# clawrim/gcn10

Hardware: AMD Instinct MI355X
Metric: CN Gpixels/sec (higher is better)
Workload: dtype u8

## Files before the change

### gcn10_amd/csrc/gcn10_gpu.hip

```cpp

#include <hip/hip_runtime.h>
#include <unistd.h>
#include <hip/hip_ext.h>

#include <cstdarg>
#include <cstdint>
#include <cstdio>
#include <cstdlib>
#include <cstring>
#include <new>

#include "gcn10_gpu.h"
#include "gcn10_gpu_internal.hpp"
#include "gcn10_soil_readers.hpp"

using gcn10::as_stream;
using gcn10::fail;
using gcn10::kLut16Bytes;
using gcn10::kLut16Plane;
using gcn10::kPlanes;
using gcn10::SoilView;
using gcn10::u32x4;
using gcn10::use_device;

namespace {

constexpr int kThreads = 256;
constexpr int kPxPerLane = 16;
constexpr int kChunk = kThreads * kPxPerLane;
constexpr int kInvalidPlane = kPlanes - 1;
constexpr int kPlane1 = 256 + 4;
constexpr int kLut1Bytes = kPlanes * kPlane1;


struct StripParams {
    const uint8_t *esa;
    SoilView soil;
    const uint8_t *lut;
    uint8_t *out[GCN10_N_RASTERS];
    uint32_t W;
    uint32_t rows;
    uint32_t npix;
    uint32_t nvec16;
    uint32_t nchunks;
    uint32_t table_mask;
    uint32_t single_k;
    uint32_t xcd_slabs;
    const uint32_t *cx;
    const uint8_t *codes;
    uint32_t codes_stride;
    const uint32_t *soil_complex;
    uint32_t soil_gen;
};

__host__ __device__ inline uint8_t soil_code(uint8_t h)
{
    uint8_t d, u;
    if (h >= 11 && h <= 14) {
        d = 4;
        u = (uint8_t)(h - 10);
    }
    else {
        d = u = (h < 5) ? h : (uint8_t)kInvalidPlane;
    }
    return (uint8_t)(d | (u << 4));
}


__device__ __forceinline__ u32x4 load16_aligned_nt(const uint8_t *p)
{
    return __builtin_nontemporal_load(reinterpret_cast<const u32x4 *>(p));
}

__device__ __forceinline__ u32x4 load16_aligned(const uint8_t *p)
{
    return *reinterpret_cast<const u32x4 *>(p);
}

__device__ __forceinline__ u32x4 load16_any(const uint8_t *p)
{
    typedef u32x4 u32x4_u __attribute__((aligned(1)));
    return *reinterpret_cast<const u32x4_u *>(p);
}

template <bool NT = true>
__device__ __forceinline__ void store16(uint8_t *p, u32x4 v)
{
    if (NT)
        __builtin_nontemporal_store(v, reinterpret_cast<u32x4 *>(p));
    else
        *reinterpret_cast<u32x4 *>(p) = v;
}

__device__ __forceinline__ int32_t scalar_load_i32(const int32_t *base, uint32_t i)
{
    typedef const int32_t __attribute__((address_space(4))) *const_ptr_t;
    const_ptr_t cp = (const_ptr_t)(uintptr_t)base;
    return cp[__builtin_amdgcn_readfirstlane(i)];
}

__device__ __forceinline__ uint32_t first_chunk(uint32_t nchunks, uint32_t &step,
                                                uint32_t &end, bool xcd_slabs)
{
    uint32_t nb = gridDim.x;
    uint32_t b = blockIdx.x;
    if (xcd_slabs && nb % 8u == 0u && nchunks >= nb) {
        uint32_t xcd = b & 7u;
        uint32_t per = (nchunks + 7u) / 8u;
        uint32_t lo = xcd * per;
        uint32_t hi = lo + per < nchunks ? lo + per : nchunks;
        step = nb / 8u;
        end = hi;
        return lo + (b >> 3);
    }
    step = nb;
    end = nchunks;
    return b;
}

enum { kLut16 = 0, kLut1 = 1 };
constexpr uint32_t kWavePx = 64u * kPxPerLane;
constexpr uint32_t kMinVectorW = kWavePx + 16u;

enum { kSoilBytes = 0, kSoilLanes = 1, kSoilPixels = 2 };

template <int ILP>
struct Trip {
    u32x4 e16[ILP], c16[ILP];
    uint32_t i0[ILP];
};

template <int ILP, bool NT>
__device__ __forceinline__ void issue_trip(const StripParams &p, uint32_t trip, uint32_t lane_off,
                                           uint32_t wave_off, Trip<ILP> &tr)
{
    uint32_t xb[ILP], r0[ILP], r1[ILP], wb[ILP];
#pragma unroll
    for (int u = 0; u < ILP; u++) {
        wb[u] = __builtin_amdgcn_readfirstlane((trip * ILP + u) * (uint32_t)kChunk + wave_off);
        const uint32_t wbc = wb[u] < p.npix ? wb[u] : 0u;
        const uint32_t y = wbc / p.W;
        xb[u] = wbc - y * p.W;
        r0[u] = (uint32_t)scalar_load_i32(p.soil.cj, y);
        r1[u] = (uint32_t)scalar_load_i32(p.soil.cj, y + 1u < p.rows ? y + 1u : y);
    }
#pragma unroll
    for (int u = 0; u < ILP; u++) {
        tr.i0[u] = wb[u] + lane_off;
        const uint8_t *pe = p.esa + (tr.i0[u] < p.nvec16 ? tr.i0[u] : 0u);
        tr.e16[u] = NT ? load16_aligned_nt(pe) : load16_aligned(pe);
    }
#pragma unroll
    for (int u = 0; u < ILP; u++) {
        uint32_t xl = xb[u] + lane_off;
        const bool wrap = xl >= p.W;
        xl = wrap ? xl - p.W : xl;
        const uint32_t row = p.soil.clamp(wrap ? r1[u] : r0[u]);
        const uint8_t *pa = p.soil.at(row, xl);
        u32x4 a = load16_any(pa);
        if (p.W & 15u) {
            const uint32_t n = p.W - xl;
            const bool strad = !wrap && n < (uint32_t)kPxPerLane;
            if (__builtin_amdgcn_ballot_w64(strad) != 0ull) {
                const uint8_t *pb = strad ? p.soil.at(p.soil.clamp(r1[u]), 0u) - n : pa;
                const u32x4 b = load16_any(pb);
                const uint32_t nn = strad ? n : (uint32_t)kPxPerLane;
#pragma unroll
                for (int j = 0; j < 4; j++) {
                    const int32_t m = (int32_t)nn - 4 * j;
                    const uint32_t mask = m >= 4 ? 0xffffffffu : (m <= 0 ? 0u : (1u << (8 * m)) - 1u);
                    a[j] = (a[j] & mask) | (b[j] & ~mask);
                }
            }
        }
        tr.c16[u] = a;
    }
}

struct LaneSoil {
    uint32_t base;
    uint32_t lim;
    uint32_t sub_px;
    uint32_t y_first;
    uint32_t B;
    bool wrap;
    uint32_t x;
    uint32_t c_lo, c_hi;
    int32_t split;
    uint32_t mask[4];
    bool pair;
};

__device__ __forceinline__ uint32_t split_mask(int32_t split, int j)
{
    const int32_t m = split - 4 * j;
    return m >= 4 ? 0xffffffffu : (m <= 0 ? 0u : (1u << (8 * m)) - 1u);
}

template <int SOIL>
__device__ __forceinline__ void lane_prologue(const StripParams &p, const gcn10::StripLanePlan &pl, LaneSoil &ls)
{
    const uint32_t g_first = __builtin_amdgcn_readfirstlane(pl.g);
    ls.base = (pl.row_lo * pl.G + pl.t) * (uint32_t)kPxPerLane;
    ls.lim = pl.active ? pl.row_hi * p.W : 0u;
    ls.sub_px = pl.B * p.W;
    ls.y_first = pl.row_lo + __builtin_amdgcn_readfirstlane(pl.rho);
    ls.B = pl.B;
    ls.wrap = pl.g < g_first;
    ls.x = pl.g * (uint32_t)kPxPerLane;
    ls.c_lo = ls.c_hi = 0u;
    ls.split = 16;
    ls.pair = true;
    if (SOIL == kSoilLanes) {
        uint32_t cx[16];
#pragma unroll
        for (int j = 0; j < 4; j++) {
            const u32x4 c4 = *reinterpret_cast<const u32x4 *>(p.cx + ls.x + 4 * j);
#pragma unroll
            for (int q = 0; q < 4; q++)
                cx[4 * j + q] = c4[q];
        }
        ls.c_lo = cx[0];
        ls.c_hi = cx[15];
        uint32_t split = 0;
#pragma unroll
        for (int q = 0; q < 16; q++)
            split += cx[q] == ls.c_lo && split == (uint32_t)q ? 1u : 0u;
        ls.split = (int32_t)split;
#pragma unroll
        for (int j = 0; j < 4; j++)
            ls.mask[j] = split_mask(ls.split, j);
        ls.pair = __builtin_amdgcn_ballot_w64(ls.c_hi - ls.c_lo > 1u) == 0ull;
    }
}

template <int ILP, bool NT, int SOIL>
__device__ __forceinline__ void issue_lane_trip(const StripParams &p, const LaneSoil &ls, uint32_t trip,
                                                Trip<ILP> &tr)
{
    uint32_t o0[ILP], o1[ILP];
#pragma unroll
    for (int u = 0; u < ILP; u++) {
        const uint32_t y = ls.y_first + (trip * ILP + u) * ls.B;
        const uint32_t ya = y < p.rows ? y : p.rows - 1u;
        const uint32_t yb = y + 1u < p.rows ? y + 1u : p.rows - 1u;
        o0[u] = p.soil.clamp((uint32_t)scalar_load_i32(p.soil.cj, ya)) * p.codes_stride;
        o1[u] = p.soil.clamp((uint32_t)scalar_load_i32(p.soil.cj, yb)) * p.codes_stride;
    }
#pragma unroll
    for (int u = 0; u < ILP; u++) {
        const uint32_t i0 = ls.base + (trip * ILP + u) * ls.sub_px;
        const bool live = i0 < ls.lim;
        tr.i0[u] = live ? i0 : 0xffffffffu;
        const uint8_t *pe = p.esa + (live ? i0 : 0u);
        tr.e16[u] = NT ? load16_aligned_nt(pe) : load16_aligned(pe);
    }
#pragma unroll
    for (int u = 0; u < ILP; u++) {
        const uint32_t off = ls.wrap ? o1[u] : o0[u];
        if (SOIL == kSoilLanes) {
            typedef uint16_t u16_u __attribute__((aligned(1)));
            tr.c16[u][0] = *reinterpret_cast<const u16_u *>(p.codes + (off + ls.c_lo));
            if (!ls.pair)
                tr.c16[u][1] = p.codes[off + ls.c_hi];
        }
        else {
            const uint8_t *cr = p.codes + off;
            const u32x4 *pc = reinterpret_cast<const u32x4 *>(p.cx + ls.x);
            u32x4 a = { 0u, 0u, 0u, 0u };
#pragma unroll 1
            for (int j = 0; j < 4; j++) {
                const u32x4 c4 = pc[j];
                const uint32_t w = (uint32_t)cr[c4[0]] | (uint32_t)cr[c4[1]] << 8 | (uint32_t)cr[c4[2]] << 16 |
                                   (uint32_t)cr[c4[3]] << 24;
                a[0] = j == 0 ? w : a[0];
                a[1] = j == 1 ? w : a[1];
                a[2] = j == 2 ? w : a[2];
                a[3] = j == 3 ? w : a[3];
            }
            tr.c16[u] = a;
        }
    }
}

template <bool KEEP_MASKS>
__device__ __forceinline__ u32x4 mix_lane_codes(const LaneSoil &ls, const u32x4 &c)
{
    const uint32_t a = (c[0] & 0xffu) * 0x01010101u;
    const uint32_t b = (ls.pair ? (c[0] >> 8) & 0xffu : c[1] & 0xffu) * 0x01010101u;
    u32x4 cd;
    int32_t split = ls.split;
    if (!KEEP_MASKS)
        asm volatile("" : "+v"(split));
#pragma unroll
    for (int j = 0; j < 4; j++) {
        const uint32_t mask = KEEP_MASKS ? ls.mask[j] : split_mask(split, j);
        cd[j] = (a & mask) | (b & ~mask);
    }
    return cd;
}

template <int KIND, int COND_MASK, int ILP, bool NT, int SOIL>
__device__ __forceinline__ void finish_trip(const StripParams &p, const uint8_t *lut, uint32_t tmask,
                                            const Trip<ILP> &tr, const LaneSoil &ls)
{
#pragma unroll
    for (int u = 0; u < ILP; u++) {
        const bool live = tr.i0[u] < p.nvec16;
        const u32x4 c16 = SOIL == kSoilLanes ? mix_lane_codes<KIND == kLut1>(ls, tr.c16[u]) : tr.c16[u];
#pragma unroll
        for (int c = 0; c < 2; c++) {
            if (!(COND_MASK & (1 << c)))
                continue;
            if (KIND == kLut16) {
                uint32_t acc[9][4];
                gcn10::gather16(lut, tr.e16[u], c16, c, acc);
                if (live) {
#pragma unroll
                    for (int k = 0; k < 9; k++) {
                        if (tmask & (1u << k)) {
                            u32x4 v = {acc[k][0], acc[k][1], acc[k][2], acc[k][3]};
                            store16<NT>(p.out[c * 9 + k] + tr.i0[u], v);
                        }
                    }
                }
            }
            else {
                u32x4 v;
#pragma unroll
                for (int j = 0; j < 4; j++) {
                    const uint32_t e = tr.e16[u][j];
                    const uint32_t cd = c16[j];
                    uint32_t w = 0;
#pragma unroll
                    for (int q = 0; q < 4; q++) {
                        const uint32_t lc = (e >> (8 * q)) & 0xffu;
                        const uint32_t s = (cd >> (8 * q + 4 * c)) & 0xfu;
                        const uint32_t b = lut[s * (uint32_t)kPlane1 + lc];
                        w |= b << (8 * q);
                    }
                    v[j] = w;
                }
                if (live)
                    store16<NT>(p.out[c * 9 + p.single_k] + tr.i0[u], v);
            }
        }
    }
}

template <int KIND, int COND_MASK, int ILP, bool NT, bool PF, int SOIL>
__device__ __forceinline__ void strip_loop(const StripParams &p, const uint8_t *lut, uint32_t tmask)
{
    uint32_t step = 1u, end, trip = 0u, lane_off = 0u, wave_off = 0u;
    LaneSoil ls = {};
    if (SOIL == kSoilBytes) {
        lane_off = (threadIdx.x & 63u) * kPxPerLane;
        wave_off = __builtin_amdgcn_readfirstlane(threadIdx.x >> 6) * kWavePx;
        trip = first_chunk(p.nchunks, step, end, p.xcd_slabs != 0);
    }
    else {
        const gcn10::StripLanePlan pl = gcn10::strip_lane_plan(p.W, p.rows, gridDim.x, blockIdx.x, threadIdx.x,
                                                               p.xcd_slabs != 0, (uint32_t)ILP);
        end = __builtin_amdgcn_readfirstlane(pl.trips);
        if (!__builtin_amdgcn_readfirstlane((uint32_t)pl.active))
            return;
        lane_prologue<SOIL>(p, pl, ls);
    }
    if (trip >= end)
        return;
    auto issue = [&](uint32_t t, Trip<ILP> &tr) {
        if (SOIL == kSoilBytes)
            issue_trip<ILP, NT>(p, t, lane_off, wave_off, tr);
        else
            issue_lane_trip<ILP, NT, SOIL>(p, ls, t, tr);
    };
    if (!PF) {
        for (; trip < end; trip += step) {
            Trip<ILP> tr;
            issue(trip, tr);
            finish_trip<KIND, COND_MASK, ILP, NT, SOIL>(p, lut, tmask, tr, ls);
        }
    }
    else {
        Trip<ILP> ta, tb;
        issue(trip, ta);
        for (;;) {
            trip += step;
            if (trip >= end) {
                finish_trip<KIND, COND_MASK, ILP, NT, SOIL>(p, lut, tmask, ta, ls);
                break;
            }
            issue(trip, tb);
            finish_trip<KIND, COND_MASK, ILP, NT, SOIL>(p, lut, tmask, ta, ls);
            trip += step;
            if (trip >= end) {
                finish_trip<KIND, COND_MASK, ILP, NT, SOIL>(p, lut, tmask, tb, ls);
                break;
            }
            issue(trip, ta);
            finish_trip<KIND, COND_MASK, ILP, NT, SOIL>(p, lut, tmask, tb, ls);
        }
    }
}

template <int KIND, int COND_MASK, bool ALL_TABLES, int ILP, bool NT, bool PF>
__global__ __launch_bounds__(kThreads) void cn_strip_kernel(const StripParams p)
{
    constexpr int kLutBytes = KIND == kLut16 ? kLut16Bytes : kLut1Bytes;
    __shared__ __attribute__((aligned(16))) uint8_t lut[kLutBytes];

    if (KIND == kLut16) {
        gcn10::stage_lut16<kThreads>(lut, p.lut);
    }
    else {
        const uint32_t *src = reinterpret_cast<const uint32_t *>(p.lut);
        uint32_t *dst = reinterpret_cast<uint32_t *>(lut);
        for (int i = threadIdx.x; i < kLutBytes / 4; i += kThreads)
            dst[i] = src[i];
    }
    __syncthreads();

    const uint32_t tmask = ALL_TABLES ? 0x1ffu : p.table_mask;

    if (!p.codes)
        strip_loop<KIND, COND_MASK, ILP, NT, PF, kSoilBytes>(p, lut, tmask);
    else if ((uint32_t)scalar_load_i32(reinterpret_cast<const int32_t *>(p.soil_complex), 0u) != p.soil_gen)
        strip_loop<KIND, COND_MASK, ILP, NT, PF, kSoilLanes>(p, lut, tmask);
    else
        strip_loop<KIND, COND_MASK, ILP, NT, PF, kSoilPixels>(p, lut, tmask);

    if (blockIdx.x == 0 && threadIdx.x < p.npix - p.nvec16) {
        const uint32_t i = p.nvec16 + threadIdx.x;
        const uint32_t y = i / p.W;
        const uint32_t x = i - y * p.W;
        const uint32_t lc = p.esa[i];
        const uint32_t cd = *p.soil.ptr(y, x);
#pragma unroll
        for (int c = 0; c < 2; c++) {
            if (!(COND_MASK & (1 << c)))
                continue;
            const uint32_t s = (cd >> (4 * c)) & 0xfu;
            if (KIND == kLut16) {
                const uint8_t *row = gcn10::lut16_row(lut, s, lc);
                for (int k = 0; k < 9; k++)
                    if (tmask & (1u << k))
                        p.out[c * 9 + k][i] = row[k];
            }
            else {
                p.out[c * 9 + p.single_k][i] = lut[s * (uint32_t)kPlane1 + lc];
            }
        }
    }
}

__global__ __launch_bounds__(kThreads) void stream_copy_kernel(const u32x4 *in, u32x4 *out, uint32_t nvec,
                                                               uint32_t ntrips)
{
    uint32_t step, end;
    for (uint32_t trip = first_chunk(ntrips, step, end, true); trip < end; trip += step) {
        u32x4 v[2];
        uint32_t idx[2];
#pragma unroll
        for (int u = 0; u < 2; u++) {
            idx[u] = (trip * 2u + u) * (uint32_t)kThreads + threadIdx.x;
            v[u] = __builtin_nontemporal_load(in + (idx[u] < nvec ? idx[u] : 0u));
        }
#pragma unroll
        for (int u = 0; u < 2; u++)
            if (idx[u] < nvec)
                __builtin_nontemporal_store(v[u], out + idx[u]);
    }
}

__global__ __launch_bounds__(kThreads) void cn_strip_bytes(const StripParams p,
                                                           uint32_t cond_mask)
{
    __shared__ __attribute__((aligned(16))) uint8_t lut[kLut16Bytes];
    gcn10::stage_lut16<kThreads>(lut, p.lut);
    __syncthreads();

    const uint32_t stride = gridDim.x * blockDim.x;
    for (uint32_t i = blockIdx.x * blockDim.x + threadIdx.x; i < p.npix; i += stride) {
        const uint32_t y = i / p.W;
        const uint32_t x = i - y * p.W;
        const uint32_t lc = p.esa[i];
        const uint32_t cd = *p.soil.ptr(y, x);
        for (int c = 0; c < 2; c++) {
            if (!(cond_mask & (1u << c)))
                continue;
            const uint32_t s = (cd >> (4 * c)) & 0xfu;
            const uint8_t *row = gcn10::lut16_row(lut, s, lc);
            for (int k = 0; k < 9; k++)
                if (p.table_mask & (1u << k))
                    p.out[c * 9 + k][i] = row[k];
        }
    }
}

template <bool VEC>
__global__ __launch_bounds__(kThreads) void soil_tables_kernel(const uint8_t *coarse, uint32_t hsx, uint32_t hsy,
                                                               const int32_t *ci, uint32_t W, uint32_t hx_stride,
                                                               uint8_t *codes, uint32_t codes_stride,
                                                               uint32_t *cx_out, uint32_t *complex, uint32_t gen)
{
    const uint32_t pad = (uint32_t)(kInvalidPlane | (kInvalidPlane << 4));
    if (blockIdx.y >= 1u) {
        const uint32_t per_row = codes_stride / 16u;
        const uint32_t t = ((blockIdx.y - 1u) * gridDim.x + blockIdx.x) * blockDim.x + threadIdx.x;
        const uint32_t r = t / per_row;
        if (r >= hsy)
            return;
        const uint32_t c0 = (t - r * per_row) * 16u;
        const uint8_t *row = coarse + (size_t)r * hsx;
        u32x4 in = { 0u, 0u, 0u, 0u };
        if (c0 + 16u <= hsx) {
            in = load16_any(row + c0);
        }
        else {
#pragma unroll
            for (int q = 0; q < 16; q++)
                if (c0 + q < hsx)
                    in[q >> 2] |= (uint32_t)row[c0 + q] << (8 * (q & 3));
        }
        u32x4 o;
#pragma unroll
        for (int j = 0; j < 4; j++) {
            uint32_t w = 0;
#pragma unroll
            for (int q = 0; q < 4; q++) {
                const uint32_t code = c0 + 4 * j + q < hsx ? soil_code((uint8_t)(in[j] >> (8 * q))) : pad;
                w |= code << (8 * q);
            }
            o[j] = w;
        }
        *reinterpret_cast<u32x4 *>(codes + (size_t)r * codes_stride + c0) = o;
        return;
    }
    const uint32_t x = (blockIdx.x * blockDim.x + threadIdx.x) * 16u;
    if (x >= hx_stride)
        return;
    uint32_t cx[16];
    if (VEC && x + 16u <= W) {
        const u32x4 *civ = reinterpret_cast<const u32x4 *>(ci + x);
#pragma unroll
        for (int j = 0; j < 4; j++) {
            const u32x4 c4 = civ[j];
#pragma unroll
            for (int q = 0; q < 4; q++)
                cx[4 * j + q] = c4[q] < hsx ? c4[q] : hsx - 1u;
        }
    }
    else {
#pragma unroll
        for (int q = 0; q < 16; q++) {
            const uint32_t xx = x + q;
            const uint32_t c = xx < W ? (uint32_t)ci[xx] : 0u;
            cx[q] = xx < W ? (c < hsx ? c : hsx - 1u) : hsx;
        }
    }
    const uint32_t c_lo = cx[0], c_hi = cx[15];
    uint32_t split = 0;
    bool compact = true;
#pragma unroll
    for (int q = 0; q < 16; q++) {
        const bool lo = cx[q] == c_lo;
        compact = compact && (lo ? split == (uint32_t)q : cx[q] == c_hi);
        split += lo && split == (uint32_t)q ? 1u : 0u;
    }
#pragma unroll
    for (int j = 0; j < 4; j++)
        *reinterpret_cast<u32x4 *>(cx_out + x + 4 * j) =
            u32x4{ cx[4 * j], cx[4 * j + 1], cx[4 * j + 2], cx[4 * j + 3] };
    if (x < W && !compact && *reinterpret_cast<volatile uint32_t *>(complex) != gen)
        *reinterpret_cast<volatile uint32_t *>(complex) = gen;
}

constexpr uint32_t kExpandRows = 4;

__global__ __launch_bounds__(kThreads) void expand_code_bytes(const uint8_t *codes, uint32_t codes_stride,
                                                              uint32_t hsy, const uint32_t *cx_in, uint8_t *hx,
                                                              uint32_t hx_stride)
{
// ... 799 lines not shown
    if (npix == 0)
        return GCN10_OK;
    if (!esa || !hsg || !out)
        return fail(GCN10_E_INVAL, "gcn10_gpu_calculate_cn: null pointer");
    const uint8_t *img = ctx->d_lut1 + (size_t)table_index * kLut1Bytes;
    const bool vec = aligned16(esa) && aligned16(hsg) && aligned16(out);
    const uint64_t work = vec ? (npix / 16 + 2 * kThreads - 1) / (2 * kThreads) + 1
                              : (npix + kThreads - 1) / kThreads;
    const uint32_t grid = stream_grid(ctx, work);
    if (vec)
        hipLaunchKernelGGL(calculate_cn_kernel<true>, dim3(grid), dim3(kThreads), 0,
                           as_stream(ctx, stream), esa, hsg, npix, img, out);
    else
        hipLaunchKernelGGL(calculate_cn_kernel<false>, dim3(grid), dim3(kThreads), 0,
                           as_stream(ctx, stream), esa, hsg, npix, img, out);
    HIP_TRY(hipGetLastError());
    return GCN10_OK;
}


int gcn10_gpu_prepare_tile(gcn10_gpu_ctx *ctx, const uint8_t *coarse, int hsx, int hsy,
                           const int32_t *ci, int W, gcn10_stream_t stream)
{
    int rc = use_device(ctx);
    if (rc)
        return rc;
    if (hsx <= 0 || hsy <= 0 || W <= 0)
        return fail(GCN10_E_INVAL, "gcn10_gpu_prepare_tile: bad shape W=%d soil=%dx%d", W, hsx, hsy);
    if (!coarse || !ci)
        return fail(GCN10_E_INVAL, "gcn10_gpu_prepare_tile: null pointer");
    const uint32_t stride = (((uint32_t)W + 15u) & ~15u) + 16u;
    const size_t need_hx = ((size_t)stride * (size_t)hsy + 63) & ~(size_t)63;
    const uint32_t codes_stride = (((uint32_t)hsx + 1u) + 15u) & ~15u;
    const size_t off_cx = (need_hx + 15) & ~(size_t)15;
    const size_t off_codes = (off_cx + (size_t)stride * 4u + 15) & ~(size_t)15;
    const size_t need = off_codes + (size_t)codes_stride * (size_t)hsy;
    if (need > ctx->hx_capacity) {
        HIP_TRY(hipDeviceSynchronize());
        if (ctx->d_hx_alloc)
            HIP_TRY(hipFree(ctx->d_hx_alloc));
        ctx->d_hx_alloc = ctx->d_hx = nullptr;
        ctx->hx_capacity = 0;
        ctx->hx_W = 0;
        HIP_TRY(hipMalloc(reinterpret_cast<void **>(&ctx->d_hx_alloc), 16 + need));
        ctx->d_hx = ctx->d_hx_alloc + 16;
        ctx->hx_capacity = need;
    }
    ctx->d_cx = reinterpret_cast<uint32_t *>(ctx->d_hx + off_cx);
    ctx->d_codes = ctx->d_hx + off_codes;
    ctx->codes_stride = codes_stride;
    if (++ctx->soil_gen == 0u)
        ctx->soil_gen = 1u;
    ctx->hx_made = false;
    ctx->hx_stride = stride;
    ctx->hx_W = (uint32_t)W;
    ctx->hx_rows = (uint32_t)hsy;
    hipStream_t s = as_stream(ctx, stream);
    const uint32_t group_blocks = (stride / 16u + kThreads - 1) / kThreads;
    const size_t code_threads = (size_t)(codes_stride / 16u) * (size_t)hsy;
    const uint32_t code_chunks = (uint32_t)((code_threads + (size_t)group_blocks * kThreads - 1) / ((size_t)group_blocks * kThreads));
    auto fn = aligned16(ci) ? soil_tables_kernel<true> : soil_tables_kernel<false>;
    hipLaunchKernelGGL(fn, dim3(group_blocks, 1u + code_chunks), dim3(kThreads), 0, s, coarse, (uint32_t)hsx,
                       (uint32_t)hsy, ci, (uint32_t)W, stride, ctx->d_codes, codes_stride, ctx->d_cx,
                       ctx->d_soil_complex, ctx->soil_gen);
    HIP_TRY(hipGetLastError());
    if (!ctx->compact_soil || (W & 15)) {
        const uint8_t *hx;
        return gcn10::soil_bytes(ctx, s, &hx);
    }
    return GCN10_OK;
}

int gcn10_gpu_cn_strip(gcn10_gpu_ctx *ctx, const uint8_t *esa, int W, int rows,
                       const int32_t *cj, unsigned cond_mask, unsigned table_mask,
                       uint8_t *const out[GCN10_N_RASTERS], gcn10_stream_t stream)
{
    int rc = use_device(ctx);
    if (rc)
        return rc;
    const char *const who = "gcn10_gpu_cn_strip";
    if ((rc = gcn10::check_tables(ctx, who)) != GCN10_OK || (rc = gcn10::check_tile(ctx, who)) != GCN10_OK)
        return rc;
    if (W <= 0 || rows < 0 || (uint32_t)W != ctx->hx_W)
        return fail(GCN10_E_INVAL, "gcn10_gpu_cn_strip: W=%d rows=%d does not match prepared tile W=%u",
                    W, rows, ctx->hx_W);
    if ((uint64_t)W * (uint64_t)rows > 0x7fffffffull)
        return fail(GCN10_E_INVAL, "gcn10_gpu_cn_strip: strip of %d x %d exceeds 2^31-1 pixels", W, rows);
    if ((rc = gcn10::check_masks(ctx, who, cond_mask, table_mask)) != GCN10_OK)
        return rc;
    if (rows == 0)
        return GCN10_OK;
    if (!esa || !cj || !out)
        return fail(GCN10_E_INVAL, "gcn10_gpu_cn_strip: null pointer");

    StripParams p;
    memset(&p, 0, sizeof p);
    bool all_aligned = aligned16(esa);
    for (int r = 0; r < GCN10_N_RASTERS; r++) {
        if (!gcn10::selected(r, cond_mask, table_mask))
            continue;
        if (!out[r])
            return fail(GCN10_E_INVAL, "gcn10_gpu_cn_strip: out[%d] is null but selected", r);
        p.out[r] = out[r];
        all_aligned = all_aligned && aligned16(out[r]);
    }
    p.esa = esa;
    p.W = (uint32_t)W;
    p.rows = (uint32_t)rows;
    p.npix = (uint32_t)((uint64_t)W * (uint64_t)rows);
    p.nchunks = (p.npix + kChunk - 1) / kChunk;
    p.table_mask = table_mask;
    hipStream_t s = as_stream(ctx, stream);

    p.xcd_slabs = (uint32_t)ctx->xcd_slabs;
    p.nvec16 = p.npix & ~15u;
    if (p.npix < 16u || p.W < kMinVectorW)
        all_aligned = false;
    const bool single = popcount(table_mask) == 1;
    const bool tuned = single && ctx->single.set;
    const int n_streams = popcount(cond_mask) * popcount(table_mask);
    const int ilp = tuned ? ctx->single.ilp
                          : single ? ctx->ilp1 : (ctx->ilp16 > 0 ? ctx->ilp16 : (n_streams > 9 ? 1 : 2));
    p.nchunks = (p.nchunks + (uint32_t)ilp - 1) / (uint32_t)ilp;
    const uint32_t grid = stream_grid(ctx, p.nchunks, tuned ? ctx->single.grid_blocks_per_cu : 0);
    if (tuned)
        p.xcd_slabs = (uint32_t)ctx->single.xcd_slabs;
    if (all_aligned && ctx->compact_soil && (p.W & 15u) == 0u &&
        gcn10::strip_lane_plan(p.W, p.rows, grid, 0u, 0u, p.xcd_slabs != 0, (uint32_t)ilp).B > 0u) {
        p.soil = SoilView{ nullptr, cj, ctx->hx_stride, ctx->hx_rows };
        p.cx = ctx->d_cx;
        p.codes = ctx->d_codes;
        p.codes_stride = ctx->codes_stride;
        p.soil_complex = ctx->d_soil_complex;
        p.soil_gen = ctx->soil_gen;
    }
    else {
        rc = gcn10::bind_soil(ctx, who, W, s, cj, &p.soil);
        if (rc)
            return rc;
    }
    if (!all_aligned) {
        p.lut = ctx->d_lut16;
        const uint32_t g = stream_grid(ctx, ((uint64_t)p.npix + kThreads - 1) / kThreads);
        void *args[] = { &p, &cond_mask };
        HIP_TRY(launch_timed(ctx, reinterpret_cast<const void *>(cn_strip_bytes), g, args, s));
        ctx->last_kernel = "cn_strip_bytes";
    }
    else {
        const bool all = table_mask == 0x1ffu;
        const bool nt = ctx->nontemporal != 0;
        if (single) {
            p.single_k = (uint32_t)__builtin_ctz(table_mask);
            p.lut = ctx->d_lut1 + (size_t)p.single_k * kLut1Bytes;
        }
        else {
            p.lut = ctx->d_lut16;
        }
        const bool pf = (tuned ? ctx->single.prefetch : ctx->prefetch) != 0 && ilp <= 2;
        strip_kernel_t fn = pick_strip_kernel(single, cond_mask, all, ilp, nt, pf);
        if (!fn)
            return fail(GCN10_E_INVAL, "gcn10_gpu_cn_strip: no kernel for ilp=%d", ilp);
        void *args[] = { &p };
        HIP_TRY(launch_timed(ctx, reinterpret_cast<const void *>(fn), grid, args, s));
        snprintf(ctx->kernel_name, sizeof ctx->kernel_name, "cn_strip_kernel<%d, %u, %s, %d, %s, %s>",
                 single ? 1 : 0, cond_mask, (all || single) ? "true" : "false", ilp, nt ? "true" : "false",
                 pf ? "true" : "false");
        ctx->last_kernel = ctx->kernel_name;
    }
    HIP_TRY(hipGetLastError());
    return GCN10_OK;
}

size_t gcn10_gpu_strip_algorithmic_bytes(int W, int rows, int hsx, int hsy, unsigned cond_mask,
                                         unsigned table_mask)
{
    if (W <= 0 || rows <= 0)
        return 0;
    const size_t n_out = (size_t)popcount(cond_mask & 3u) * (size_t)popcount(table_mask & 0x1ffu);
    return (size_t)W * rows * (1 + n_out) + (size_t)(hsx > 0 ? hsx : 0) * (hsy > 0 ? hsy : 0) +
           4 * ((size_t)W + rows);
}

int gcn10_gpu_set_option(gcn10_gpu_ctx *ctx, const char *name, int value)
{
    if (!ctx || !name)
        return fail(GCN10_E_INVAL, "gcn10_gpu_set_option: null argument");
    if (!strcmp(name, "defaults")) {
        const gcn10_gpu_ctx fresh;
        ctx->grid_blocks_per_cu = fresh.grid_blocks_per_cu;
        ctx->ilp16 = fresh.ilp16;
        ctx->ilp1 = fresh.ilp1;
        ctx->nontemporal = fresh.nontemporal;
        ctx->xcd_slabs = fresh.xcd_slabs;
        ctx->prefetch = fresh.prefetch;
        ctx->compact_soil = fresh.compact_soil;
        ctx->deflate_wave_codes = fresh.deflate_wave_codes;
        ctx->arena_segment_align = fresh.arena_segment_align;
        ctx->fused_parse = fresh.fused_parse;
        ctx->fused_emit = fresh.fused_emit;
        ctx->event_sync_sleep_us = fresh.event_sync_sleep_us;
        ctx->single = fresh.single;
    }
    else if (!strcmp(name, "grid_blocks_per_cu") && value >= 1 && value <= 64)
        ctx->grid_blocks_per_cu = value;
    else if (!strcmp(name, "ilp16") && (value == 0 || value == 1 || value == 2))
        ctx->ilp16 = value;
    else if (!strcmp(name, "ilp1") && (value == 1 || value == 2 || value == 4)) {
        ctx->ilp1 = value;
        ctx->single.set = false;
    }
    else if (!strcmp(name, "nontemporal") && (value == 0 || value == 1))
        ctx->nontemporal = value;
    else if (!strcmp(name, "xcd_slabs") && (value == 0 || value == 1))
        ctx->xcd_slabs = value;
    else if (!strcmp(name, "deflate_wave_codes") && (value == 0 || value == 1))
        ctx->deflate_wave_codes = value;
    else if (!strcmp(name, "arena_segment_align") && value >= 16 && value <= 4096 && (value & (value - 1)) == 0)
        ctx->arena_segment_align = value;
    else if (!strcmp(name, "fused_emit") && (value == 0 || value == 1))
        ctx->fused_emit = value;
    else if (!strcmp(name, "fused_parse") && (value == 0 || value == 1))
        ctx->fused_parse = value;
    else if (!strcmp(name, "event_sync_sleep_us") && value >= 0 && value <= 100000)
        ctx->event_sync_sleep_us = value;
    else if (!strcmp(name, "prefetch") && (value == -1 || value == 0 || value == 1))
        ctx->prefetch = value;
    else if (!strcmp(name, "compact_soil") && (value == 0 || value == 1))
        ctx->compact_soil = value;
    else
        return fail(GCN10_E_INVAL, "gcn10_gpu_set_option: unknown option or bad value: %s=%d", name, value);
    return GCN10_OK;
}

int gcn10_gpu_time_next_strip(gcn10_gpu_ctx *ctx, gcn10_event_t start, gcn10_event_t stop)
{
    if (!ctx || !start || !stop)
        return fail(GCN10_E_INVAL, "gcn10_gpu_time_next_strip: null argument");
    ctx->time_start = reinterpret_cast<hipEvent_t>(start);
    ctx->time_stop = reinterpret_cast<hipEvent_t>(stop);
    return GCN10_OK;
}

int gcn10_gpu_stream_copy(gcn10_gpu_ctx *ctx, const void *src, void *dst, size_t bytes, gcn10_stream_t stream)
{
    int rc = use_device(ctx);
    if (rc)
        return rc;
    if (bytes == 0)
        return GCN10_OK;
    if (!src || !dst || (bytes & 15u) || !aligned16(src) || !aligned16(dst) || bytes / 16 > 0x7fffffffull)
        return fail(GCN10_E_INVAL, "gcn10_gpu_stream_copy: needs 16-byte aligned pointers and size (< 32 GiB)");
    const u32x4 *in = static_cast<const u32x4 *>(src);
    u32x4 *out = static_cast<u32x4 *>(dst);
    uint32_t nvec = (uint32_t)(bytes / 16);
    uint32_t ntrips = (nvec + 2u * kThreads - 1u) / (2u * kThreads);
    const uint32_t grid = stream_grid(ctx, ntrips);
    hipStream_t s = as_stream(ctx, stream);
    void *args[] = { &in, &out, &nvec, &ntrips };
    HIP_TRY(launch_timed(ctx, reinterpret_cast<const void *>(stream_copy_kernel), grid, args, s));
    HIP_TRY(hipGetLastError());
    return GCN10_OK;
}

int gcn10_gpu_tune_single_raster(gcn10_gpu_ctx *ctx, const uint8_t *esa, int W, int rows, const int32_t *cj,
                                 unsigned cond_mask, unsigned table_mask, uint8_t *arena, size_t arena_bytes,
                                 size_t step, uint8_t **best_out, float *best_ms, char *report, size_t report_cap,
                                 gcn10_stream_t stream)
{
    int rc = use_device(ctx);
    if (rc)
        return rc;
    if (!best_out || !arena || !esa || !cj)
        return fail(GCN10_E_INVAL, "gcn10_gpu_tune_single_raster: null pointer");
    if (popcount(cond_mask & 3u) != 1 || popcount(table_mask & 0x1ffu) != 1 || (cond_mask & ~3u) || (table_mask >> 9))
        return fail(GCN10_E_INVAL, "gcn10_gpu_tune_single_raster: exactly one condition and one table");
    if (W <= 0 || rows <= 0 || (uint64_t)W * (uint64_t)rows > 0x7fffffffull)
        return fail(GCN10_E_INVAL, "gcn10_gpu_tune_single_raster: bad shape %d x %d", W, rows);
    const size_t npix = (size_t)W * (size_t)rows;
    if (step == 0 || (step & 255u) || !aligned16(arena) || arena_bytes < npix)
        return fail(GCN10_E_INVAL, "gcn10_gpu_tune_single_raster: arena of %zu bytes / step %zu cannot hold a raster of %zu",
                    arena_bytes, step, npix);
    const int r = (cond_mask & 2u ? 9 : 0) + __builtin_ctz(table_mask);
    struct Shape { int xcd, bpc, ilp, pf; };
    static const Shape shapes[] = { {1, 8, 2, 1}, {1, 16, 2, 1}, {1, 8, 4, 0}, {1, 16, 4, 0}, {1, 16, 1, 0}, {1, 8, 2, 0},
                                    {1, 16, 2, 0}, {1, 8, 1, 1} };
    const gcn10_gpu_ctx::SingleShape saved = ctx->single;
    hipStream_t s = as_stream(ctx, stream);
    constexpr int kRuns = 3;
    hipEvent_t e0[kRuns], e1[kRuns];
    for (int i = 0; i < kRuns; i++) {
        e0[i] = e1[i] = nullptr;
        if (hipEventCreate(&e0[i]) != hipSuccess || hipEventCreate(&e1[i]) != hipSuccess)
            return fail(GCN10_E_HIP, "gcn10_gpu_tune_single_raster: event creation failed");
    }
    float best = 1e30f, worst = 0.f;
    size_t best_pos = 0;
    Shape best_shape = shapes[0];
    int n_pos = 0;
    rc = GCN10_OK;
    for (size_t pos = 0; pos + npix <= arena_bytes && rc == GCN10_OK; pos += step, n_pos++) {
        uint8_t *out[GCN10_N_RASTERS] = { nullptr };
        out[r] = arena + pos;
        for (const Shape &sh : shapes) {
            ctx->single.set = true;
            ctx->single.xcd_slabs = sh.xcd;
            ctx->single.grid_blocks_per_cu = sh.bpc;
// ... 75 lines not shown
```

Measured before the change: 2968.

## Overlap LUT staging with early soil and landcover loads in strip kernel

Splits the strip loop into a code-bytes path and a soil-tables path. The soil-tables path issues row-index, column and first-trip landcover loads before staging the LUT into LDS, and software-pipelines the row-pair loads and code offsets one trip ahead. Offsets and row values are pinned to scalar registers, the lane-code byte broadcast uses perm with an xor-select blend, and per-condition single-table output pointers are precomputed on the host. The goal is to hide global-load latency behind LUT staging and the previous trip. The cost is more register pressure and more complex control flow, and the soil path now returns before the scalar tail-pixel handling.

New measurement: 2971, median of 3. About the same (+0.1%).

```diff
diff --git a/gcn10_amd/csrc/gcn10_gpu.hip b/gcn10_amd/csrc/gcn10_gpu.hip
--- a/gcn10_amd/csrc/gcn10_gpu.hip
+++ b/gcn10_amd/csrc/gcn10_gpu.hip
@@ -9,6 +9,7 @@
 #include <cstdlib>
 #include <cstring>
 #include <new>
+#include <type_traits>
 
 #include "gcn10_gpu.h"
 #include "gcn10_gpu_internal.hpp"
@@ -45,6 +46,7 @@
     uint32_t nchunks;
     uint32_t table_mask;
     uint32_t single_k;
+    uint8_t *out1[2];
     uint32_t xcd_slabs;
     const uint32_t *cx;
     const uint8_t *codes;
@@ -97,6 +99,15 @@
     typedef const int32_t __attribute__((address_space(4))) *const_ptr_t;
     const_ptr_t cp = (const_ptr_t)(uintptr_t)base;
     return cp[__builtin_amdgcn_readfirstlane(i)];
+}
+
+__device__ __forceinline__ void scalar_load_row_pair(const int32_t *base, uint32_t y, uint32_t rows, int32_t &a,
+                                                     int32_t &b)
+{
+    typedef const int32_t __attribute__((address_space(4))) *const_ptr_t;
+    const_ptr_t cp = (const_ptr_t)(uintptr_t)base;
+    a = cp[y < rows ? y : rows - 1u];
+    b = cp[y + 1u < rows ? y + 1u : rows - 1u];
 }
 
 __device__ __forceinline__ uint32_t first_chunk(uint32_t nchunks, uint32_t &step,
@@ -197,67 +208,102 @@
     return m >= 4 ? 0xffffffffu : (m <= 0 ? 0u : (1u << (8 * m)) - 1u);
 }
 
-template <int SOIL>
-__device__ __forceinline__ void lane_prologue(const StripParams &p, const gcn10::StripLanePlan &pl, LaneSoil &ls)
+__device__ __forceinline__ void lane_plan(const StripParams &p, const gcn10::StripLanePlan &pl, LaneSoil &ls)
 {
     const uint32_t g_first = __builtin_amdgcn_readfirstlane(pl.g);
     ls.base = (pl.row_lo * pl.G + pl.t) * (uint32_t)kPxPerLane;
     ls.lim = pl.active ? pl.row_hi * p.W : 0u;
-    ls.sub_px = pl.B * p.W;
-    ls.y_first = pl.row_lo + __builtin_amdgcn_readfirstlane(pl.rho);
-    ls.B = pl.B;
+    ls.B = __builtin_amdgcn_readfirstlane(pl.B);
+    ls.sub_px = ls.B * p.W;
+    ls.y_first = __builtin_amdgcn_readfirstlane(pl.row_lo + pl.rho);
     ls.wrap = pl.g < g_first;
     ls.x = pl.g * (uint32_t)kPxPerLane;
     ls.c_lo = ls.c_hi = 0u;
     ls.split = 16;
     ls.pair = true;
-    if (SOIL == kSoilLanes) {
-        uint32_t cx[16];
-#pragma unroll
-        for (int j = 0; j < 4; j++) {
-            const u32x4 c4 = *reinterpret_cast<const u32x4 *>(p.cx + ls.x + 4 * j);
-#pragma unroll
-            for (int q = 0; q < 4; q++)
-                cx[4 * j + q] = c4[q];
-        }
-        ls.c_lo = cx[0];
-        ls.c_hi = cx[15];
-        uint32_t split = 0;
-#pragma unroll
-        for (int q = 0; q < 16; q++)
-            split += cx[q] == ls.c_lo && split == (uint32_t)q ? 1u : 0u;
-        ls.split = (int32_t)split;
-#pragma unroll
-        for (int j = 0; j < 4; j++)
-            ls.mask[j] = split_mask(ls.split, j);
-        ls.pair = __builtin_amdgcn_ballot_w64(ls.c_hi - ls.c_lo > 1u) == 0ull;
-    }
-}
-
-template <int ILP, bool NT, int SOIL>
-__device__ __forceinline__ void issue_lane_trip(const StripParams &p, const LaneSoil &ls, uint32_t trip,
-                                                Trip<ILP> &tr)
-{
-    uint32_t o0[ILP], o1[ILP];
+}
+
+__device__ __forceinline__ void load_lane_columns(const StripParams &p, const LaneSoil &ls, u32x4 cx[4])
+{
+#pragma unroll
+    for (int j = 0; j < 4; j++)
+        cx[j] = *reinterpret_cast<const u32x4 *>(p.cx + ls.x + 4 * j);
+}
+
+__device__ __forceinline__ void lane_column_entry(const u32x4 cx[4], LaneSoil &ls)
+{
+    ls.c_lo = cx[0][0];
+    ls.c_hi = cx[3][3];
+    uint32_t split = 0;
+#pragma unroll
+    for (int q = 0; q < 16; q++)
+        split += cx[q >> 2][q & 3] == ls.c_lo && split == (uint32_t)q ? 1u : 0u;
+    ls.split = (int32_t)split;
+#pragma unroll
+    for (int j = 0; j < 4; j++)
+        ls.mask[j] = split_mask(ls.split, j);
+    ls.pair = __builtin_amdgcn_ballot_w64(ls.c_hi - ls.c_lo > 1u) == 0ull;
+}
+
+template <int ILP>
+struct TripRows {
+    int32_t a[ILP], b[ILP];
+};
+
+template <int ILP>
+__device__ __forceinline__ void load_trip_rows(const StripParams &p, const LaneSoil &ls, uint32_t trip,
+                                               TripRows<ILP> &rw)
+{
+#pragma unroll
+    for (int u = 0; u < ILP; u++)
+        scalar_load_row_pair(p.soil.cj, ls.y_first + (trip * ILP + u) * ls.B, p.rows, rw.a[u], rw.b[u]);
+}
+
+template <int ILP, bool NT>
+__device__ __forceinline__ void issue_lane_landcover(const StripParams &p, const LaneSoil &ls, uint32_t trip,
+                                                     Trip<ILP> &tr)
+{
 #pragma unroll
     for (int u = 0; u < ILP; u++) {
-        const uint32_t y = ls.y_first + (trip * ILP + u) * ls.B;
-        const uint32_t ya = y < p.rows ? y : p.rows - 1u;
-        const uint32_t yb = y + 1u < p.rows ? y + 1u : p.rows - 1u;
-        o0[u] = p.soil.clamp((uint32_t)scalar_load_i32(p.soil.cj, ya)) * p.codes_stride;
-        o1[u] = p.soil.clamp((uint32_t)scalar_load_i32(p.soil.cj, yb)) * p.codes_stride;
-    }
-#pragma unroll
-    for (int u = 0; u < ILP; u++) {
-        const uint32_t i0 = ls.base + (trip * ILP + u) * ls.sub_px;
+        uint32_t sub = __builtin_amdgcn_readfirstlane((trip * ILP + u) * ls.sub_px);
+        asm("" : "+s"(sub));
+        const uint32_t i0 = ls.base + sub;
         const bool live = i0 < ls.lim;
         tr.i0[u] = live ? i0 : 0xffffffffu;
         const uint8_t *pe = p.esa + (live ? i0 : 0u);
         tr.e16[u] = NT ? load16_aligned_nt(pe) : load16_aligned(pe);
     }
+}
+
+template <int ILP>
+struct TripOffsets {
+    uint32_t o0[ILP], o1[ILP];
+};
+
+template <int ILP, bool PINNED>
+__device__ __forceinline__ void trip_offsets(const StripParams &p, TripRows<ILP> &rw, TripOffsets<ILP> &of)
+{
 #pragma unroll
     for (int u = 0; u < ILP; u++) {
-        const uint32_t off = ls.wrap ? o1[u] : o0[u];
+        if (PINNED) {
+            rw.a[u] = __builtin_amdgcn_readfirstlane(rw.a[u]);
+            rw.b[u] = __builtin_amdgcn_readfirstlane(rw.b[u]);
+            asm volatile("" : "+s"(rw.a[u]), "+s"(rw.b[u]) : : "memory");
+        }
+        of.o0[u] = __builtin_amdgcn_readfirstlane(p.soil.clamp((uint32_t)rw.a[u]) * p.codes_stride);
+        of.o1[u] = __builtin_amdgcn_readfirstlane(p.soil.clamp((uint32_t)rw.b[u]) * p.codes_stride);
+        asm("" : "+s"(of.o0[u]), "+s"(of.o1[u]));
+    }
+}
+
+template <int ILP, int SOIL>
+__device__ __forceinline__ void issue_lane_codes(const StripParams &p, const LaneSoil &ls,
+                                                 const TripOffsets<ILP> &of, Trip<ILP> &tr)
+{
+#pragma unroll
+    for (int u = 0; u < ILP; u++) {
+        const uint32_t o0 = of.o0[u], o1 = of.o1[u];
+        const uint32_t off = ls.wrap ? o1 : o0;
         if (SOIL == kSoilLanes) {
             typedef uint16_t u16_u __attribute__((aligned(1)));
             tr.c16[u][0] = *reinterpret_cast<const u16_u *>(p.codes + (off + ls.c_lo));
@@ -286,8 +332,8 @@
 template <bool KEEP_MASKS>
 __device__ __forceinline__ u32x4 mix_lane_codes(const LaneSoil &ls, const u32x4 &c)
 {
-    const uint32_t a = (c[0] & 0xffu) * 0x01010101u;
-    const uint32_t b = (ls.pair ? (c[0] >> 8) & 0xffu : c[1] & 0xffu) * 0x01010101u;
+    const uint32_t a = gcn10::perm(c[0], c[0], 0x00000000u);
+    const uint32_t b = ls.pair ? gcn10::perm(c[0], c[0], 0x01010101u) : gcn10::perm(c[1], c[1], 0x00000000u);
     u32x4 cd;
     int32_t split = ls.split;
     if (!KEEP_MASKS)
@@ -295,7 +341,7 @@
 #pragma unroll
     for (int j = 0; j < 4; j++) {
         const uint32_t mask = KEEP_MASKS ? ls.mask[j] : split_mask(split, j);
-        cd[j] = (a & mask) | (b & ~mask);
+        cd[j] = b ^ ((a ^ b) & mask);
     }
     return cd;
 }
@@ -342,64 +388,144 @@
                     v[j] = w;
                 }
                 if (live)
-                    store16<NT>(p.out[c * 9 + p.single_k] + tr.i0[u], v);
+                    store16<NT>(p.out1[c] + tr.i0[u], v);
             }
         }
     }
 }
 
-template <int KIND, int COND_MASK, int ILP, bool NT, bool PF, int SOIL>
-__device__ __forceinline__ void strip_loop(const StripParams &p, const uint8_t *lut, uint32_t tmask)
-{
-    uint32_t step = 1u, end, trip = 0u, lane_off = 0u, wave_off = 0u;
-    LaneSoil ls = {};
-    if (SOIL == kSoilBytes) {
-        lane_off = (threadIdx.x & 63u) * kPxPerLane;
-        wave_off = __builtin_amdgcn_readfirstlane(threadIdx.x >> 6) * kWavePx;
-        trip = first_chunk(p.nchunks, step, end, p.xcd_slabs != 0);
+template <int ILP, bool PF, class Issue, class Finish>
+__device__ __forceinline__ void strip_trips(Trip<ILP> &ta, uint32_t trip, uint32_t end, uint32_t step, Issue issue,
+                                            Finish finish)
+{
+    if (!PF) {
+        finish(ta);
+        for (trip += step; trip < end; trip += step) {
+            issue(trip, ta);
+            finish(ta);
+        }
     }
     else {
-        const gcn10::StripLanePlan pl = gcn10::strip_lane_plan(p.W, p.rows, gridDim.x, blockIdx.x, threadIdx.x,
-                                                               p.xcd_slabs != 0, (uint32_t)ILP);
-        end = __builtin_amdgcn_readfirstlane(pl.trips);
-        if (!__builtin_amdgcn_readfirstlane((uint32_t)pl.active))
-            return;
-        lane_prologue<SOIL>(p, pl, ls);
-    }
+        Trip<ILP> tb;
+        for (trip += step; trip + step < end; trip += 2u * step) {
+            issue(trip, tb);
+            finish(ta);
+            issue(trip + step, ta);
+            finish(tb);
+        }
+        if (trip < end) {
+            issue(trip, tb);
+            finish(ta);
+            finish(tb);
+        }
+        else {
+            finish(ta);
+        }
+    }
+}
+
+template <int KIND>
+struct StagedLut {
+    typedef typename std::conditional<KIND == kLut16, u32x4, uint32_t>::type word_t;
+    static constexpr int kBytes = KIND == kLut16 ? kLut16Bytes : kLut1Bytes;
+    static constexpr int kWords = kBytes / (int)sizeof(word_t);
+    static constexpr int kSteps = (kWords + kThreads - 1) / kThreads;
+    word_t regs[kSteps];
+
+    __device__ __forceinline__ void load(const uint8_t *src)
+    {
+#pragma unroll
+        for (int k = 0; k < kSteps; k++) {
+            const int i = k * kThreads + (int)threadIdx.x;
+            if ((k + 1) * kThreads <= kWords || i < kWords)
+                regs[k] = reinterpret_cast<const word_t *>(src)[i];
+        }
+    }
+    __device__ __forceinline__ void store(uint8_t *lds) const
+    {
+#pragma unroll
+        for (int k = 0; k < kSteps; k++) {
+            const int i = k * kThreads + (int)threadIdx.x;
+            if ((k + 1) * kThreads <= kWords || i < kWords)
+                reinterpret_cast<word_t *>(lds)[i] = regs[k];
+        }
+    }
+};
+
+template <int KIND, int COND_MASK, int ILP, bool NT, bool PF>
+__device__ __forceinline__ void strip_of_code_bytes(const StripParams &p, uint8_t *lut, uint32_t tmask)
+{
+    StagedLut<KIND> image;
+    image.load(p.lut);
+    image.store(lut);
+    __syncthreads();
+    const LaneSoil ls = {};
+    const uint32_t lane_off = (threadIdx.x & 63u) * kPxPerLane;
+    const uint32_t wave_off = __builtin_amdgcn_readfirstlane(threadIdx.x >> 6) * kWavePx;
+    uint32_t step, end;
+    const uint32_t trip = first_chunk(p.nchunks, step, end, p.xcd_slabs != 0);
     if (trip >= end)
         return;
-    auto issue = [&](uint32_t t, Trip<ILP> &tr) {
-        if (SOIL == kSoilBytes)
-            issue_trip<ILP, NT>(p, t, lane_off, wave_off, tr);
-        else
-            issue_lane_trip<ILP, NT, SOIL>(p, ls, t, tr);
+    Trip<ILP> ta;
+    issue_trip<ILP, NT>(p, trip, lane_off, wave_off, ta);
+    strip_trips<ILP, PF>(
+        ta, trip, end, step, [&](uint32_t t, Trip<ILP> &tr) { issue_trip<ILP, NT>(p, t, lane_off, wave_off, tr); },
+        [&](const Trip<ILP> &tr) { finish_trip<KIND, COND_MASK, ILP, NT, kSoilBytes>(p, lut, tmask, tr, ls); });
+}
+
+template <int KIND, int COND_MASK, int ILP, bool NT, bool PF>
+__device__ __forceinline__ void strip_of_soil_tables(const StripParams &p, uint8_t *lut, uint32_t tmask)
+{
+    const gcn10::StripLanePlan pl = gcn10::strip_lane_plan(p.W, p.rows, gridDim.x, blockIdx.x, threadIdx.x,
+                                                           p.xcd_slabs != 0, (uint32_t)ILP);
+    if (__builtin_amdgcn_readfirstlane(pl.t - threadIdx.x) >= pl.B * pl.G)
+        return;
+    const uint32_t end = __builtin_amdgcn_readfirstlane(pl.trips);
+    LaneSoil ls;
+    lane_plan(p, pl, ls);
+    const uint32_t complex_word = (uint32_t)scalar_load_i32(reinterpret_cast<const int32_t *>(p.soil_complex), 0u);
+    TripRows<ILP> rows0, rows1;
+    load_trip_rows<ILP>(p, ls, 0u, rows0);
+    load_trip_rows<ILP>(p, ls, 1u, rows1);
+    constexpr bool kEarlyLandcover = ILP == 1;
+    Trip<ILP> ta;
+    if (kEarlyLandcover)
+        issue_lane_landcover<ILP, NT>(p, ls, 0u, ta);
+    u32x4 cx[4];
+    load_lane_columns(p, ls, cx);
+    StagedLut<KIND> image;
+    image.load(p.lut);
+    image.store(lut);
+    __syncthreads();
+    if (!kEarlyLandcover)
+        issue_lane_landcover<ILP, NT>(p, ls, 0u, ta);
+    if (!__builtin_amdgcn_readfirstlane((uint32_t)pl.active) || end == 0u)
+        return;
+
+    TripOffsets<ILP> of;
+    trip_offsets<ILP, false>(p, rows0, of);
+    auto lane_trips = [&](auto soil) {
+        constexpr int SOIL = decltype(soil)::value;
+        issue_lane_codes<ILP, SOIL>(p, ls, of, ta);
+        trip_offsets<ILP, false>(p, rows1, of);
+        strip_trips<ILP, PF>(
+            ta, 0u, end, 1u,
+            [&](uint32_t t, Trip<ILP> &tr) {
+                load_trip_rows<ILP>(p, ls, t + 1u, rows1);
+                issue_lane_landcover<ILP, NT>(p, ls, t, tr);
+                issue_lane_codes<ILP, SOIL>(p, ls, of, tr);
+            },
+            [&](const Trip<ILP> &tr) {
+                finish_trip<KIND, COND_MASK, ILP, NT, SOIL>(p, lut, tmask, tr, ls);
+                trip_offsets<ILP, true>(p, rows1, of);
+            });
     };
-    if (!PF) {
-        for (; trip < end; trip += step) {
-            Trip<ILP> tr;
-            issue(trip, tr);
-            finish_trip<KIND, COND_MASK, ILP, NT, SOIL>(p, lut, tmask, tr, ls);
-        }
+    if (complex_word != p.soil_gen) {
+        lane_column_entry(cx, ls);
+        lane_trips(std::integral_constant<int, kSoilLanes>());
     }
     else {
-        Trip<ILP> ta, tb;
-        issue(trip, ta);
-        for (;;) {
-            trip += step;
-            if (trip >= end) {
-                finish_trip<KIND, COND_MASK, ILP, NT, SOIL>(p, lut, tmask, ta, ls);
-                break;
-            }
-            issue(trip, tb);
-            finish_trip<KIND, COND_MASK, ILP, NT, SOIL>(p, lut, tmask, ta, ls);
-            trip += step;
-            if (trip >= end) {
-                finish_trip<KIND, COND_MASK, ILP, NT, SOIL>(p, lut, tmask, tb, ls);
-                break;
-            }
-            issue(trip, ta);
-            finish_trip<KIND, COND_MASK, ILP, NT, SOIL>(p, lut, tmask, tb, ls);
-        }
+        lane_trips(std::integral_constant<int, kSoilPixels>());
     }
 }
 
@@ -408,26 +534,13 @@
 {
     constexpr int kLutBytes = KIND == kLut16 ? kLut16Bytes : kLut1Bytes;
     __shared__ __attribute__((aligned(16))) uint8_t lut[kLutBytes];
-
-    if (KIND == kLut16) {
-        gcn10::stage_lut16<kThreads>(lut, p.lut);
-    }
-    else {
-        const uint32_t *src = reinterpret_cast<const uint32_t *>(p.lut);
-        uint32_t *dst = reinterpret_cast<uint32_t *>(lut);
-        for (int i = threadIdx.x; i < kLutBytes / 4; i += kThreads)
-            dst[i] = src[i];
-    }
-    __syncthreads();
-
     const uint32_t tmask = ALL_TABLES ? 0x1ffu : p.table_mask;
 
-    if (!p.codes)
-        strip_loop<KIND, COND_MASK, ILP, NT, PF, kSoilBytes>(p, lut, tmask);
-    else if ((uint32_t)scalar_load_i32(reinterpret_cast<const int32_t *>(p.soil_complex), 0u) != p.soil_gen)
-        strip_loop<KIND, COND_MASK, ILP, NT, PF, kSoilLanes>(p, lut, tmask);
-    else
-        strip_loop<KIND, COND_MASK, ILP, NT, PF, kSoilPixels>(p, lut, tmask);
+    if (p.codes) {
+        strip_of_soil_tables<KIND, COND_MASK, ILP, NT, PF>(p, lut, tmask);
+        return;
+    }
+    strip_of_code_bytes<KIND, COND_MASK, ILP, NT, PF>(p, lut, tmask);
 
     if (blockIdx.x == 0 && threadIdx.x < p.npix - p.nvec16) {
         const uint32_t i = p.nvec16 + threadIdx.x;
@@ -1533,6 +1646,8 @@
         if (single) {
             p.single_k = (uint32_t)__builtin_ctz(table_mask);
             p.lut = ctx->d_lut1 + (size_t)p.single_k * kLut1Bytes;
+            p.out1[0] = p.out[p.single_k];
+            p.out1[1] = p.out[9 + p.single_k];
         }
         else {
             p.lut = ctx->d_lut16;
```
